# ShuvalovIvan/RayTracingProject

Hardware: AMD Instinct MI355X
Metric: Mrays/sec + frame time, random-spheres 1920x1080x256spp (higher is better)
Workload: dtype f32

## Files before the change

raytracingproject_amd/build.py:

```python
from __future__ import annotations

import os
import subprocess
from concurrent.futures import ThreadPoolExecutor
from pathlib import Path

PKG = Path(__file__).resolve().parent
ROOT = PKG.parent
CSRC = PKG / "csrc"
OBJ = PKG / "build"
LIB = PKG / "lib" / "librt_hip.so"
ARCH = os.environ.get("RT_OFFLOAD_ARCH", "gfx950")
HIPCC = os.environ.get("HIPCC", "/opt/rocm/bin/hipcc")

COMMON = ["-x", "hip", f"--offload-arch={ARCH}", "-O3", "-std=c++17", "-fPIC", "-Wall",
          "-Wno-unused-function", f"-I{ROOT / 'include'}"] + os.environ.get("RT_HIPCC_EXTRA", "").split()
F32_FAST = ["-fno-hip-fp32-correctly-rounded-divide-sqrt", "-fgpu-flush-denormals-to-zero",
            os.environ.get("RT_F32_CONTRACT", "-ffp-contract=on")]
UNITS = {
    "rt_render_f32.hip": F32_FAST,
    "rt_query_grid_f32.hip": F32_FAST,
    "rt_render_f64.hip": ["-ffp-contract=off"],
    "rt_abi.cpp": ["-ffp-contract=off"],
    "rt_plan.cpp": ["-ffp-contract=off"],
# ... 7 lines not shown
HEADERS = ["rt_device.h", "rt_render_impl.h", "rt_occluded.h", "rt_radiance.h", "rt_pixels.h", "rt_moments.h", "rt_aov.h", "rt_scene.h", "rt_launch.h", "rt_bvh.h", "rt_lbvh.h", "rt_ctx.h", "rt_devbuf.h",
           "rt_treelet.h", "rt_pack.h", "rt_batch_cull.h", "rt_denoise.h", "rt_quant.h"]


def _stale(target: Path, deps: list[Path]) -> bool:
    if not target.exists():
        return True
    t = target.stat().st_mtime
    return any(d.stat().st_mtime > t for d in deps)


def _present(p: Path) -> bool:
    try:
        return p.exists()
    except OSError:
        return False


def _compile(src: str, extra: list[str], verbose: bool) -> Path:
    obj = OBJ / (src.rsplit(".", 1)[0] + ".o")
    deps = [CSRC / src] + [CSRC / h for h in HEADERS] + [ROOT / "include" / "rt_hip.h", Path(__file__)]
    if _stale(obj, deps):
        cmd = [HIPCC, *COMMON, *extra, "-c", str(CSRC / src), "-o", str(obj)]
        if verbose:
            print(" ".join(cmd), flush=True)
        subprocess.run(cmd, check=True)
    return obj


def build_native(verbose: bool = False) -> Path:
    OBJ.mkdir(parents=True, exist_ok=True)
    LIB.parent.mkdir(parents=True, exist_ok=True)
    with ThreadPoolExecutor(max_workers=4) as ex:
        objs = list(ex.map(lambda kv: _compile(kv[0], kv[1], verbose), UNITS.items()))
    if _stale(LIB, objs):
        cmd = [HIPCC, f"--offload-arch={ARCH}", "-shared", "-fPIC", "-o", str(LIB), *map(str, objs),
               "-L/opt/rocm/lib", "-lrccl", "-Wl,-rpath,/opt/rocm/lib"]
        if verbose:
            print(" ".join(cmd), flush=True)
        subprocess.run(cmd, check=True)
    return LIB


def build_dropin(verbose: bool = False) -> list[Path]:
    out_dir = ROOT / "examples" / "_build"
    out_dir.mkdir(parents=True, exist_ok=True)
    inc = ROOT / "include" / "rt"
    link = [f"-L{LIB.parent}", "-lrt_hip", f"-Wl,-rpath,{LIB.parent}", "-Wl,-rpath,$ORIGIN/../../raytracingproject_amd/lib"]
    built = []
    for name in ("pixelmatch", "host_queries", "mesh_scene"):
        exe = out_dir / name
        src = ROOT / "examples" / f"{name}.cpp"
        if _stale(exe, [src, LIB, *inc.glob("*.h")]):
            subprocess.run(["g++", "-O2", "-std=c++17", f"-I{inc}", str(src), "-o", str(exe), *link], check=True)
        built.append(exe)
    ref_main = Path("/root/reference/src/main.cpp")
    if _present(ref_main):
        exe = out_dir / "reference_main_on_mi355x"
        if _stale(exe, [ref_main, LIB, *inc.glob("*.h")]):
            with open(ref_main, "rb") as f:
                subprocess.run(["g++", "-O2", "-std=c++17", "-x", "c++", "-", f"-I{inc}", "-o", str(exe), *link],
                               check=True, stdin=f, cwd=inc)
        built.append(exe)
    return built


SAN_FLAGS = ["-O1", "-g", "-fno-omit-frame-pointer", "-fsanitize=address,undefined",
             "-fno-sanitize-recover=all"]
SAN_EXE = OBJ / "san" / "san_driver"
INC = f"-I{ROOT / 'include'}"


def _build_san(exe: Path, srcs: list[Path], deps: list[Path], extra=(), verbose: bool = False) -> Path:
    exe.parent.mkdir(parents=True, exist_ok=True)
    if _stale(exe, [*srcs, *deps, Path(__file__)]):
        cmd = ["g++", "-std=c++17", *SAN_FLAGS, *extra, *map(str, srcs), "-o", str(exe), "-lm"]
        if verbose:
            print(" ".join(cmd), flush=True)
        subprocess.run(cmd, check=True)
    return exe


def build_sanitize(verbose: bool = False) -> Path:
    SAN_EXE.parent.mkdir(parents=True, exist_ok=True)
    orc, oo = ROOT / "oracle" / "rt_oracle.c", SAN_EXE.parent / "rt_oracle.o"
    if _stale(oo, [orc, ROOT / "oracle" / "rt_oracle.h", Path(__file__)]):
        cmd = ["gcc", "-std=c11", *SAN_FLAGS, "-c", str(orc), "-o", str(oo)]
        if verbose:
            print(" ".join(cmd), flush=True)
        subprocess.run(cmd, check=True)
    srcs = [ROOT / "tests" / "cpp" / "sanitize_driver.cpp", CSRC / "rt_obj.cpp", CSRC / "rt_bvh.cpp", oo]
    deps = [CSRC / "rt_bvh.h", CSRC / "rt_scene.h", ROOT / "include" / "rt_hip.h", ROOT / "oracle" / "rt_oracle.h"]
    return _build_san(SAN_EXE, srcs, deps, [INC], verbose)


RESUME_EXE = OBJ / "san" / "grid_resume_driver"
BOXES_EXE = OBJ / "san" / "bvh_boxes_driver"
PACK_EXE = OBJ / "san" / "pack_driver"
DEVBUF_EXE = OBJ / "san" / "devbuf_driver"
BVH_DEPS = [CSRC / "rt_bvh.h", CSRC / "rt_scene.h", ROOT / "include" / "rt_hip.h"]


def build_grid_resume(verbose: bool = False) -> Path:
    srcs = [ROOT / "tests" / "cpp" / "grid_resume_driver.cpp", CSRC / "rt_bvh.cpp"]
    return _build_san(RESUME_EXE, srcs, BVH_DEPS, ["-ffp-contract=off", INC], verbose)


def build_bvh_boxes(verbose: bool = False) -> Path:
    srcs = [ROOT / "tests" / "cpp" / "bvh_boxes_driver.cpp", CSRC / "rt_bvh.cpp"]
    return _build_san(BOXES_EXE, srcs, BVH_DEPS, ["-ffp-contract=off", INC], verbose)


def build_pack(verbose: bool = False) -> Path:
    srcs = [ROOT / "tests" / "cpp" / "pack_driver.cpp", CSRC / "rt_pack.cpp", CSRC / "rt_bvh.cpp"]
    return _build_san(PACK_EXE, srcs, [CSRC / "rt_pack.h", *BVH_DEPS], ["-ffp-contract=off", INC], verbose)


def build_devbuf(verbose: bool = False) -> Path:
    extra = ["-D__HIP_PLATFORM_AMD__", f"-I{CSRC}", "-I/opt/rocm/include"]
    return _build_san(DEVBUF_EXE, [ROOT / "tests" / "cpp" / "devbuf_driver.cpp"], [CSRC / "rt_devbuf.h"], extra, verbose)


QUANT_EXE = OBJ / "san" / "quant_range_driver"


def build_quant_range(verbose: bool = False) -> Path:
    src = ROOT / "tests" / "cpp" / "quant_range_driver.cpp"
    QUANT_EXE.parent.mkdir(parents=True, exist_ok=True)
    if _stale(QUANT_EXE, [src, CSRC / "rt_quant.h", CSRC / "rt_scene.h", Path(__file__)]):
        cmd = ["g++", "-std=c++17", "-O2", "-Wall", "-pthread", f"-I{CSRC}", INC, str(src), "-o", str(QUANT_EXE)]
        if verbose:
            print(" ".join(cmd), flush=True)
        subprocess.run(cmd, check=True)
    return QUANT_EXE


CULL_EXE = OBJ / "san" / "batch_cull_driver"
CULL_MUTANTS = (1, 2, 3)


def build_batch_cull(verbose: bool = False) -> list[Path]:
    src = ROOT / "tests" / "cpp" / "batch_cull_driver.cpp"
    deps = [CSRC / "rt_batch_cull.h", CSRC / "rt_scene.h"]
    exes = [CULL_EXE] + [CULL_EXE.with_name(f"batch_cull_driver_m{m}") for m in CULL_MUTANTS]

    def one(k: int) -> None:
        _build_san(exes[k], [src], deps, ["-O2", "-ffp-contract=off", f"-DRT_CULL_MUTATE={k}", f"-I{CSRC}"], verbose)

    with ThreadPoolExecutor(max_workers=4) as ex:
        list(ex.map(one, range(len(exes))))
    return exes


def build_oracle(verbose: bool = False) -> None:
    oracle = ROOT / "oracle"
    out = None if verbose else subprocess.DEVNULL
    subprocess.run(["make", "-C", str(oracle), "liboracle.so", "rt_oracle_cli", "ref-if-present"], check=True,
                   stdout=out)


if __name__ == "__main__":
    import sys
    if "--sanitize" in sys.argv[1:]:
        print(build_sanitize(verbose=True))
        sys.exit(0)
    print(build_native(verbose=True))
    print(build_dropin(verbose=True))
    build_oracle(verbose=True)
```

raytracingproject_amd/csrc/rt_batch_cull.h:

```cpp
#pragma once
#include <cmath>
#include <cstddef>
#include <cstdint>

#include "rt_scene.h"

namespace rtx {

constexpr int BATCH_CAND_CAP = 24;
constexpr size_t BATCH_CAND_BYTES = 128;
static_assert((BATCH_CAND_CAP + 1) * 4 <= BATCH_CAND_BYTES, "candidate list");

#ifndef RT_CULL_MUTATE
#define RT_CULL_MUTATE 0
#endif
#if RT_CULL_MUTATE == 1
constexpr float CULL_EPS = 0x1p-29f, CULL_EPS_CAM = 0x1p-31f, CULL_UP = 1.f;
#else
constexpr float CULL_EPS = 0x1p-17f, CULL_EPS_CAM = 0x1p-19f, CULL_UP = 1.f + 0x1p-19f;
#endif

struct CullBeam {
    float c[3], ax[3];
    float rl, g, scale;
    bool ok;
};

RT_HD inline CullBeam cull_beam(const float* cam, int defocus, int tx0, int ty0) {
    auto nrm = [](const float* v) { return sqrtf(v[0] * v[0] + v[1] * v[1] + v[2] * v[2]); };
    auto l1 = [](const float* v) { return fabsf(v[0]) + fabsf(v[1]) + fabsf(v[2]); };
    const float* c = cam;
    const float *p00 = cam + 3, *du = cam + 6, *dv = cam + 9, *ddu = cam + 12, *ddv = cam + 15;
    const float fx = (float)tx0 + 3.5f, fy = (float)ty0 + 3.5f;
    CullBeam b;
    float a[3];
    for (int k = 0; k < 3; ++k) {
        b.c[k] = c[k];
        a[k] = (p00[k] + fx * du[k] + fy * dv[k]) - c[k];
    }
    const float L = nrm(a);
    const float iL = 1.f / L;
    for (int k = 0; k < 3; ++k) b.ax[k] = a[k] * iL;
    b.scale = l1(c) + l1(p00) + (fx + 4.5f) * l1(du) + (fy + 4.5f) * l1(dv) + l1(ddu) + l1(ddv);
    const float E = CULL_EPS_CAM * b.scale;
    const float rho = 4.f * (nrm(du) + nrm(dv)) * CULL_UP + E;
#if RT_CULL_MUTATE == 2
    b.rl = E;
#else
    b.rl = (defocus ? nrm(ddu) + nrm(ddv) : 0.f) * CULL_UP + E;
#endif
    const float k = (b.rl + rho) * iL * CULL_UP;
    b.ok = k <= 0.875f;
    b.g = k / (1.f - k) * CULL_UP * CULL_UP;
    return b;
}

RT_HD inline bool cull_keep(const CullBeam& b, const SphereF& s) {
    const float hx = 0.5f * s.cv[0], hy = 0.5f * s.cv[1], hz = 0.5f * s.cv[2];
#if RT_CULL_MUTATE == 3
    const float rb = fabsf(s.r);
#else
    const float rb = fabsf(s.r) + sqrtf(hx * hx + hy * hy + hz * hz) * CULL_UP;
#endif
    const float qx = (s.c[0] + hx) - b.c[0], qy = (s.c[1] + hy) - b.c[1], qz = (s.c[2] + hz) - b.c[2];
    const float qn = sqrtf(qx * qx + qy * qy + qz * qz);
    const float sa = qx * b.ax[0] + qy * b.ax[1] + qz * b.ax[2];
    const float px = qx - sa * b.ax[0], py = qy - sa * b.ax[1], pz = qz - sa * b.ax[2];
    const float perp = sqrtf(px * px + py * py + pz * pz);
    const float W = (rb + b.rl) + CULL_EPS * (qn + b.scale + rb);
    const float bound = (W + b.g * fmaxf(sa + W, 0.f)) * CULL_UP;
    const bool behind = sa < -W, outside = perp > bound;
    return !b.ok || !(behind || outside);
}

RT_HD inline bool batch_cull_keep(const float* cam, int defocus, int tx0, int ty0, const SphereF& s) {
    return cull_keep(cull_beam(cam, defocus, tx0, ty0), s);
}

}
```

raytracingproject_amd/csrc/rt_device.h:

```cpp
#pragma once
#include <type_traits>
#include <hip/hip_runtime.h>

#include <cstdint>

#include "rt_scene.h"
#include "rt_batch_cull.h"
#include "rt_quant.h"


namespace rtx {

__host__ __device__ __forceinline__ uint32_t hash32(uint32_t x) {
    x ^= x >> 16;
    x *= 0x21f0aaadu;
    x ^= x >> 15;
    x *= 0xd35a2d97u;
    x ^= x >> 15;
    return x;
}
__host__ __device__ __forceinline__ uint32_t seed32_of(uint64_t seed) {
    return hash32((uint32_t)seed ^ hash32((uint32_t)(seed >> 32)));
}
constexpr uint32_t RNG_GOLDEN = 0x9e3779b9u;
// ... 35 lines not shown

__device__ __forceinline__ float rcp(float x) { return __builtin_amdgcn_rcpf(x); }
__device__ __forceinline__ double rcp(double x) { return 1.0 / x; }
__device__ __forceinline__ float slab_rcp(float x) { return rcp(x + copysignf(0x1p-100f, x)); }
__device__ __forceinline__ double slab_rcp(double x) { return rcp(x); }

template <class R>
struct V3 {
    R x, y, z;
};
template <class R> __device__ __forceinline__ V3<R> mk(R x, R y, R z) { return V3<R>{x, y, z}; }
template <class R> __device__ __forceinline__ V3<R> operator+(V3<R> a, V3<R> b) { return {a.x + b.x, a.y + b.y, a.z + b.z}; }
template <class R> __device__ __forceinline__ V3<R> operator-(V3<R> a, V3<R> b) { return {a.x - b.x, a.y - b.y, a.z - b.z}; }
template <class R> __device__ __forceinline__ V3<R> operator*(V3<R> a, V3<R> b) { return {a.x * b.x, a.y * b.y, a.z * b.z}; }
template <class R> __device__ __forceinline__ V3<R> operator-(V3<R> a) { return {-a.x, -a.y, -a.z}; }
template <class R> __device__ __forceinline__ V3<R> scl(R t, V3<R> v) { return {t * v.x, t * v.y, t * v.z}; }
template <class R> __device__ __forceinline__ V3<R> dvs(V3<R> v, R t) { return scl(rcp(t), v); }
__device__ __forceinline__ V3<float> madd(float t, V3<float> v, V3<float> c) {
    return {__builtin_fmaf(t, v.x, c.x), __builtin_fmaf(t, v.y, c.y), __builtin_fmaf(t, v.z, c.z)};
}
__device__ __forceinline__ V3<double> madd(double t, V3<double> v, V3<double> c) { return c + scl(t, v); }
template <class R> __device__ __forceinline__ R dot(V3<R> a, V3<R> b) { return a.x * b.x + a.y * b.y + a.z * b.z; }
template <class R> __device__ __forceinline__ V3<R> cross(V3<R> u, V3<R> v) {
    return {u.y * v.z - u.z * v.y, u.z * v.x - u.x * v.z, u.x * v.y - u.y * v.x};
}
template <class R> __device__ __forceinline__ R len2(V3<R> v) { return v.x * v.x + v.y * v.y + v.z * v.z; }
template <class R> __device__ __forceinline__ V3<R> unit(V3<R> v) { return dvs(v, (R)sqrt(len2(v))); }
template <class R> __device__ __forceinline__ V3<R> reflect(V3<R> v, V3<R> n) {
    if constexpr (sizeof(R) == 4) return madd(-2.f * dot(v, n), n, v);
    return v - scl((R)2 * dot(v, n), n);
}
template <class R>
__device__ __forceinline__ V3<R> refract(V3<R> uv, V3<R> n, R e) {
    R cos_theta = fmin(dot(-uv, n), (R)1.0);
    V3<R> perp = scl(e, madd(cos_theta, n, uv));
    V3<R> par = scl(-(R)sqrt(fabs((R)1.0 - len2(perp))), n);
    return perp + par;
}
template <class R, class S> __device__ __forceinline__ V3<R> cvt(V3<S> v) { return {(R)v.x, (R)v.y, (R)v.z}; }
template <class R> __device__ __forceinline__ V3<R> ld3(const double* p) { return {(R)p[0], (R)p[1], (R)p[2]}; }
template <class R> __device__ __forceinline__ V3<R> ld3(const float* p) { return {(R)p[0], (R)p[1], (R)p[2]}; }

constexpr int MAX_PHASES = 8;
struct RenderParams {
    int W, H, spp, max_depth;
    int sample_begin;
    int accumulate;
    int shard, nshards, tiles_x, shard_tiles;
    uint32_t seed32;
    int n_nodes, n_spheres, n_mats, n_big;
    int n_front;
    int stack_size;
    int defocus;
    double cam_center[3], p00[3], du[3], dv[3], ddu[3], ddv[3];
    float f_center[3], f_p00[3], f_du[3], f_dv[3], f_ddu[3], f_ddv[3];
    const Node* nodes;
    const void* spheres;
    const void* mats;
    const SphereD* big;
    const BigF* bigf;
    const Node4* mnodes;
    const void* tris;
    const uint32_t* tmeta;
    int n_mnodes;
    int mstack;
    void* out_sums;
    uint32_t* out_segs;
    unsigned long long* diag;
    void* samples;
    long long* accum;
    uint32_t* accum_flags;
    unsigned long long* accp;
    uint32_t* queue;
    int max_wgs;
    int nph;
    int ph_s0[MAX_PHASES], ph_c[MAX_PHASES], ph_k[MAX_PHASES];
    int coh_refill;
    float box_extent;
    float mbox[6];
    GridHdr grid;
    double tiles_x_inv, tiles_x_inv_half;
    int gsus_lanes, gsus_iters;
    int batch_cap, batch_adopt;
};
constexpr int GSUS_DEFAULT_LANES = 16, GSUS_DEFAULT_ITERS = 8;
constexpr size_t QUEUE_CTRL_BYTES = 4096;
constexpr int FIX_SHIFT = 28;
constexpr int FIX_SAMPLE_SHIFT = 19;
constexpr int FIX_ITEM_SAMPLES = 32;
constexpr int FIX_LAUNCH_SAMPLES = 8191;
constexpr uint32_t FIX_NAN = 1u, FIX_POS = 2u, FIX_NEG = 4u;
__device__ __forceinline__ long long fix_sample(float l, int c, uint32_t& fl, float* r_out = nullptr) {
    constexpr float SC = (float)(1 << FIX_SAMPLE_SHIFT), ISC = 1.f / SC;
    const float r = __builtin_rintf(l * SC);
    if (r_out) *r_out = r;
    const float v = r * ISC;
    if (v == 0.f) return 0;
    const double q = (double)v * (double)(1ll << FIX_SHIFT);
    if (fabs(q) < 0x1p62) return (long long)q;
    fl |= (q != q ? FIX_NAN : q > 0 ? FIX_POS : FIX_NEG) << (3 * c);
    return 0;
}
constexpr int DIAG_SLOTS = 42;

constexpr int COH_FIFO = 128;
template <bool MESH>
struct CohEntryT {
    float t;
    uint32_t pix;
    uint32_t sid;
};
template <>
struct CohEntryT<true> {
    float t;
    uint32_t pix;
    uint32_t sid;
    int32_t id;
};
using CohEntry = CohEntryT<false>;
static_assert(sizeof(CohEntryT<false>) == 12 && sizeof(CohEntryT<true>) == 16, "CohEntry");
template <bool MESH>
struct CohEntryD {
    double t;
    uint32_t pix;
    uint32_t sid;
};
template <>
struct CohEntryD<true> {
    double t;
    uint32_t pix;
    uint32_t sid;
    int32_t id;
    uint32_t pad;
};
static_assert(sizeof(CohEntryD<false>) == 16 && sizeof(CohEntryD<true>) == 24, "CohEntryD");
#ifndef RT_FIFO_RNG0
#define RT_FIFO_RNG0 1
#endif
#ifndef RT_CAM_ONEBASE
#define RT_CAM_ONEBASE 1
#endif
#ifndef RT_LEAN_FINISH
#define RT_LEAN_FINISH 1
#endif
#ifndef RT_SCATTER_PROLOGUE
#define RT_SCATTER_PROLOGUE 1
#endif
#ifndef RT_BATCH_ONEADOPT
#define RT_BATCH_ONEADOPT 1
#endif
#ifndef RT_POP_THROUGH
#define RT_POP_THROUGH 1
#endif
struct alignas(16) CohEntryR {
    float t;
    uint32_t pix;
    uint32_t sid;
    uint32_t rng0;
};
static_assert(sizeof(CohEntryR) == 16 && alignof(CohEntryR) == 16, "CohEntryR");
template <class R, bool MESH, bool RNG0> struct CohEntrySel { using type = CohEntryT<MESH>; };
template <bool MESH, bool RNG0> struct CohEntrySel<double, MESH, RNG0> { using type = CohEntryD<MESH>; };
template <> struct CohEntrySel<float, false, true> { using type = CohEntryR; };
template <class R, bool MESH, bool RNG0 = false> using CohEntryX = typename CohEntrySel<R, MESH, RNG0>::type;
constexpr size_t COH_SUM_BYTES = 64 * 3 * sizeof(float);
constexpr size_t COH_PARK_BYTES = 64 * 4 * sizeof(float);
constexpr size_t coh_wave_bytes(bool mesh, bool sums, int fifo = COH_FIFO, bool f64 = false, bool park = false,
                                bool cand = false) {
    const size_t entry = f64                    ? (mesh ? sizeof(CohEntryD<true>) : sizeof(CohEntryD<false>))
                         : cand && RT_FIFO_RNG0 ? sizeof(CohEntryR)
                                                : (mesh ? sizeof(CohEntryT<true>) : sizeof(CohEntryT<false>));
    return (size_t)fifo * entry +
           (sums && !f64 ? COH_SUM_BYTES : 0) + (park ? COH_PARK_BYTES : 0) + (cand ? BATCH_CAND_BYTES : 0);
}
constexpr size_t COH_WAVE_BYTES = coh_wave_bytes(false, true);
struct CohConst {
    float cam[18];
    int nph;
    int ph_s0[MAX_PHASES], ph_c[MAX_PHASES], ph_k[MAX_PHASES];
    int pad;
};
static_assert(sizeof(CohConst) % 16 == 0, "CohConst");
constexpr size_t COH_CAM_BYTES = sizeof(CohConst);


template <class R> struct Prec;
template <> struct Prec<float> { using Sph = SphereF; using Mat = MatF; using Tri = TriF; };
template <> struct Prec<double> { using Sph = SphereD; using Mat = MatD; using Tri = TriD; };

template <class R>
struct SceneView {
    const Node* nodes;
    const typename Prec<R>::Sph* sph;
    const typename Prec<R>::Mat* mat;
    const SphereD* big;
    const BigF* bigf;
    int n_nodes, n_big, n_front;
    const Node4* mnodes;
    const typename Prec<R>::Tri* tris;
    const uint32_t* tmeta;
    int n_mnodes;
    uint32_t* mstack;
    int n_mstack;
    float mbox[6];
    GridHdr grid;
    const __attribute__((address_space(4))) GridHdr* gridp;
    float box_extent;
};

template <class R>
struct Ray {
    V3<R> o, d;
    R time;
};

template <class T, bool EXACT, bool SELECT = false>
__device__ __forceinline__ bool sphere_root(V3<T> c, T r, V3<T> cv, bool moving, V3<T> o, V3<T> d, T a, T inv_a,
                                            T time, T tmin, T tmax, bool self, T& t) {
    V3<T> center = c;
    if (EXACT) {
        if (moving) center = c + scl(time, cv);
    } else {
        center = madd(time, cv, c);
    }
    if (EXACT) {
        V3<T> oc = o - center;
        T half_b = dot(oc, d);
        T cc = len2(oc) - r * r;
        T disc = half_b * half_b - a * cc;
        if (disc < 0) return false;
        T sq = (T)sqrt(disc);
        T root = (-half_b - sq) / a;
        if (!(tmin < root && root < tmax)) {
            root = (-half_b + sq) / a;
            if (!(tmin < root && root < tmax)) return false;
        }
        t = root;
        return true;
    }
    const V3<T> f = o - center;
    const T b = -dot(f, d);
    T root;
    if (self) {
        root = (T)2 * b * inv_a;
        if (!(tmin < root && root < tmax)) return false;
        t = root;
        return true;
    }
    const V3<T> l = madd(b * inv_a, d, f);
    const T r2 = r * r;
    const T disc = r2 - len2(l);
    if (disc < 0) return false;
    const T cc = len2(f) - r2;
    const T q = b + copysign((T)sqrt(a * disc), b);
    const T ta = cc * rcp(q), tb = q * inv_a;
    const T t0 = fmin(ta, tb), t1 = fmax(ta, tb);
    if (SELECT) {
        root = (tmin < t0 && t0 < tmax) ? t0 : t1;
        t = root;
        return tmin < root && root < tmax;
    }
    root = t0;
    if (!(tmin < root && root < tmax)) {
        root = t1;
        if (!(tmin < root && root < tmax)) return false;
    }
    t = root;
    return true;
}

template <class T>
__device__ __forceinline__ bool tri_root(V3<T> v0, V3<T> e1, V3<T> e2, V3<T> o, V3<T> d, T tmin, T tmax, T& t) {
    constexpr T EPS = (T)0;
    const V3<T> pv = cross(d, e2);
    const T det = dot(e1, pv);
    if (det == (T)0) return false;
    const T inv_det = rcp(det);
    const V3<T> tv = o - v0;
    const T u = dot(tv, pv) * inv_det;
    if (u < -EPS || u > (T)1 + EPS) return false;
    const V3<T> qv = cross(tv, e1);
    const T v = dot(d, qv) * inv_det;
    if (v < -EPS || u + v > (T)1 + EPS) return false;
    const T tt = dot(e2, qv) * inv_det;
    if (!(tmin < tt && tt < tmax)) return false;
    t = tt;
    return true;
}

__device__ __forceinline__ void vfence(float& x) { asm volatile("" : "+v"(x)); }
__device__ __forceinline__ bool tri_wt(V3<float> p0, V3<float> p1, V3<float> p2, V3<float> n, V3<float> o,
                                       V3<float> d, float tmin, float tmax, float& t) {
    const float nd = dot(n, d);
    float Ax, Ay, Az;
    {
#pragma clang fp contract(off)
        Ax = p0.x - o.x, Ay = p0.y - o.y, Az = p0.z - o.z;
    }
    const float tt = dot(n, mk(Ax, Ay, Az)) * rcp(nd);
    if (!(tmin < tt && tt < tmax)) return false;
    auto outside = [nd](float e) { return nd > 0.f ? e < 0.f : e > 0.f; };
    {
#pragma clang fp contract(off)
        const float Bx = p1.x - o.x, By = p1.y - o.y, Bz = p1.z - o.z;
        float ec = d.x * (Ay * Bz - Az * By) + d.y * (Az * Bx - Ax * Bz) + d.z * (Ax * By - Ay * Bx);
        vfence(ec);
// ... 56 lines not shown
    double tn = fmax(fmax(fmin(t0x, t1x), fmin(t0y, t1y)), fmax(fmin(t0z, t1z), tmin));
    double tf = fmin(fmin(fmax(t0x, t1x), fmax(t0y, t1y)), fmin(fmax(t0z, t1z), tmax));
    tnear = tn;
    return tn <= tf;
}

struct ConsSlabs {
    float f[3], clo[3], chi[3];
};
__device__ __forceinline__ ConsSlabs cons_slabs(V3<double> o, V3<double> d, float extent) {
    ConsSlabs s;
    const double oo[3] = {o.x, o.y, o.z}, dd[3] = {d.x, d.y, d.z};
#pragma unroll
    for (int a = 0; a < 3; ++a) {
        if (fabs(dd[a]) < 0x1p-60) {
            s.f[a] = 0.f;
            s.clo[a] = -__builtin_huge_valf();
            s.chi[a] = __builtin_huge_valf();
            continue;
        }
        const float f = (float)(1.0 / dd[a]);
        const float m = (float)((fabs(oo[a]) + (double)extent) * 0x1p-21 * fabs((double)f));
        const float c = -((float)oo[a] * f);
        s.f[a] = f;
        s.clo[a] = f > 0.f ? c - m : c + m;
        s.chi[a] = f > 0.f ? c + m : c - m;
    }
    return s;
}
__device__ __forceinline__ bool box_hit_cons(const float lo[3], const float hi[3], const ConsSlabs& s, float tmin,
                                             float tmax, float& tnear) {
    const float t0x = __builtin_fmaf(lo[0], s.f[0], s.clo[0]), t1x = __builtin_fmaf(hi[0], s.f[0], s.chi[0]);
    const float t0y = __builtin_fmaf(lo[1], s.f[1], s.clo[1]), t1y = __builtin_fmaf(hi[1], s.f[1], s.chi[1]);
    const float t0z = __builtin_fmaf(lo[2], s.f[2], s.clo[2]), t1z = __builtin_fmaf(hi[2], s.f[2], s.chi[2]);
    const float tn = fmaxf(fmaxf(fminf(t0x, t1x), fminf(t0y, t1y)), fmaxf(fminf(t0z, t1z), tmin));
    const float tf = fminf(fminf(fmaxf(t0x, t1x), fmaxf(t0y, t1y)), fmaxf(t0z, t1z));
    tnear = tn;
    return tn <= tf && tn <= tmax;
}
constexpr float CONS_TMIN = 0.0009f;
__device__ __forceinline__ float cons_tmax(double tmax) { return (float)tmax * (1.f + 0x1p-22f); }

enum { TRAV_SELROOT = 8, TRAV_B128 = 16, TRAV_F32BOX = 32, TRAV_COH = 64, TRAV_NOSUM = 128, TRAV_TBIN = 256,
       TRAV_CULL = 512, TRAV_PERSIST = 2048, TRAV_MTOP = 4096, TRAV_MIFIF = 8192, TRAV_MWHILE = 16384,
       TRAV_MQ = 32768, TRAV_GRID = 65536, TRAV_GFLAT = 131072,
       TRAV_G3D = 262144 };
constexpr int TRAV_REMOVED = TRAV_TBIN | TRAV_MTOP;
constexpr int coh_fifo_entries(int) { return COH_FIFO; }
constexpr bool coh_parks(bool mesh, int tr, bool f64) { return mesh && !f64 && (tr & TRAV_GRID) != 0; }
constexpr bool coh_cands(bool mesh, int tr, bool f64) { return !mesh && !f64 && (tr & TRAV_GRID) != 0; }
constexpr bool coh_adopts(bool mesh, int tr, bool f64) { return coh_cands(mesh, tr, f64); }
constexpr bool coh_rng0(bool mesh, int tr, bool f64) { return RT_FIFO_RNG0 && coh_cands(mesh, tr, f64); }
constexpr bool coh_cam1(bool mesh, int tr, bool f64) { return RT_CAM_ONEBASE && coh_cands(mesh, tr, f64); }
constexpr bool coh_lean(bool mesh, int tr, bool f64) { return RT_LEAN_FINISH && coh_cands(mesh, tr, f64); }
constexpr bool coh_refl1(bool mesh, int tr, bool f64) {
    return RT_SCATTER_PROLOGUE && coh_cands(mesh, tr, f64) && (tr & TRAV_GFLAT) != 0;
}
constexpr bool coh_adopt1(bool mesh, int tr, bool f64) { return RT_BATCH_ONEADOPT && coh_cands(mesh, tr, f64); }
constexpr bool coh_popthru(bool mesh, int tr, bool f64) { return RT_POP_THROUGH && coh_cands(mesh, tr, f64); }
typedef __attribute__((address_space(3))) const uint32_t lds_cu32;
typedef __attribute__((address_space(3))) const float4 lds_cf4;
__device__ __forceinline__ void keep_live(uint32_t v) { asm volatile("" ::"v"(v)); }
template <class R, bool EXACT, bool DIAG = false, int TRAV = 0, bool MESH = false, bool SUSP = false,
          bool CAND = false>
__device__ __forceinline__ Hit<R> closest_hit(const SceneView<R>& sc, const Ray<R>& ray, uint16_t* stack, int stride,
                                              int self_id, DiagCounters* dg = nullptr, float* resume = nullptr,
                                              const Hit<R>* part = nullptr, int sus_lanes = 0, int sus_iters = 0,
                                              uint32_t clist = 0, int ncand = 0) {
    static_assert(!SUSP || (!EXACT && !MESH && (TRAV & TRAV_GRID) != 0 && (TRAV & TRAV_GFLAT) != 0),
                  "resumable walks: the fp32 sphere-only flat grid walk");
    static_assert(!CAND || (!SUSP && coh_cands(MESH, TRAV, EXACT)), "candidate lists: the fp32 sphere-grid kernels");
    constexpr R TMIN = (R)0.001;
    Hit<R> h;
    h.id = -1;
    h.td = __builtin_huge_val();
    R tmax = (R)__builtin_huge_valf();
    const V3<R> o = ray.o, d = ray.d;
    const R a = len2(d);
    const R inv_a = rcp(a);
    [[maybe_unused]] bool resumed = false;
    [[maybe_unused]] float t_from = -1.f;
    if constexpr (SUSP) {
        t_from = *resume;
        *resume = -1.f;
        resumed = t_from >= 0.f;
        if (resumed) {
            h.id = part->id;
            tmax = part->t;
        }
    }

    if (SUSP && resumed) {
    } else if (EXACT) {
        const V3<double> od = cvt<double>(o), dd = cvt<double>(d);
        double tmaxd = __builtin_huge_val();
        for (int k = 0; k < sc.n_big; ++k) {
            const SphereD& s = sc.big[k];
            double t;
            if (sphere_root<double, true>(mk(s.c[0], s.c[1], s.c[2]), s.r, mk(s.cv[0], s.cv[1], s.cv[2]),
                                          (s.meta >> 30) & 1u, od, dd, (double)a, 0.0, (double)ray.time, 0.001,
                                          tmaxd, false, t)) {
                tmaxd = t;
                h.id = -2 - k;
                h.td = t;
            }
        }
        if (h.id != -1) tmax = (R)h.td;
    } else {
        for (int k = 0; k < sc.n_big; ++k) {
            const BigF& s = sc.bigf[k];
            V3<R> p0 = mk((R)s.p0[0], (R)s.p0[1], (R)s.p0[2]);
            if ((s.meta >> 30) & 1u) p0 = madd((R)ray.time, mk((R)s.cv[0], (R)s.cv[1], (R)s.cv[2]), p0);
            const V3<R> q = o - p0, nn = mk((R)s.n[0], (R)s.n[1], (R)s.n[2]);
            const R b = -fma((R)s.r, dot(nn, d), dot(q, d));
            R t;
            if ((-2 - k) == self_id) {
                t = (R)2 * b * inv_a;
                if (!(TMIN < t && t < tmax)) continue;
            } else {
                const R cc = fma((R)2 * (R)s.r, dot(nn, q), dot(q, q));
                const R disc = b * b - a * cc;
                if (disc < 0) continue;
                const R qq = b + copysign((R)sqrt(disc), b);
                const R ta = cc * rcp(qq), tb = qq * inv_a;
                const R t0 = fmin(ta, tb), t1 = fmax(ta, tb);
                t = t0;
                if (!(TMIN < t && t < tmax)) {
                    t = t1;
                    if (!(TMIN < t && t < tmax)) continue;
                }
            }
            tmax = t;
            h.id = -2 - k;
        }
    }

    using Sph = typename Prec<R>::Sph;
    auto test_rec = [&](const Sph* rec, bool is_self, R tlim, R& tk) -> bool {
        if constexpr (!EXACT && (TRAV & TRAV_B128) != 0) {
            const float4* q = (const float4*)rec;
            const float4 s0 = q[0], s1 = q[1];
            keep_live(__float_as_uint(s0.w));
            keep_live(__float_as_uint(s1.w));
            return sphere_root<R, false, (TRAV & TRAV_SELROOT) != 0>(
                mk((R)s0.x, (R)s0.y, (R)s0.z), (R)s0.w, mk((R)s1.x, (R)s1.y, (R)s1.z), false, o, d, a, inv_a,
                ray.time, TMIN, tlim, is_self, tk);
        }
        const auto& s = *rec;
        return sphere_root<R, EXACT, (TRAV & TRAV_SELROOT) != 0>(mk((R)s.c[0], (R)s.c[1], (R)s.c[2]), (R)s.r,
                                     mk((R)s.cv[0], (R)s.cv[1], (R)s.cv[2]), (s.meta >> 30) & 1u, o, d, a, inv_a,
                                     ray.time, TMIN, tlim, !EXACT && is_self, tk);
    };
    auto test_one = [&](int k, R tlim, R& tk) -> bool { return test_rec(sc.sph + k, k == self_id, tlim, tk); };
    if constexpr (CAND) {
        uint32_t hit_off = 0xffffffffu;
        for (int i = 0; i < ncand; ++i) {
            if (DIAG) DiagCounters::count(dg->leaf_it, dg->leaf_act), ++dg->steps;
            const uint32_t off = (uint32_t)__builtin_amdgcn_readfirstlane(
                (int)*(const lds_cu32*)(uintptr_t)(clist + 4u * (uint32_t)i));
            const Sph* rec = (const Sph*)(const float4*)(const lds_cf4*)(uintptr_t)off;
            R t;
            if (test_rec(rec, false, tmax, t)) {
                tmax = t;
                hit_off = off;
            }
        }
        if (hit_off != 0xffffffffu)
            h.id = (int)((hit_off - (uint32_t)sc.n_nodes * (uint32_t)sizeof(Node)) / (uint32_t)sizeof(Sph));
        h.t = tmax;
        return h;
    }
    for (int k = 0; k < (SUSP && resumed ? 0 : sc.n_front); ++k) {
        R t;
        if (test_one(k, tmax, t)) {
            tmax = t;
            h.id = k;
        }
    }

    if constexpr ((TRAV & TRAV_GRID) != 0) {
        if (sc.n_nodes > 0) {
            constexpr bool FLAT = (TRAV & TRAV_GFLAT) != 0;
            const GridHdr g = [&]() {
                if constexpr (!MESH) {
                    auto gp = sc.gridp;
                    asm volatile("" : "+s"(gp));
                    return *(const GridHdr*)gp;
                } else {
                    return sc.grid;
                }
            }();
            const uint32_t pad = (uint32_t)g.res[0] * (uint32_t)g.res[1];
            const uint32_t* cells = (const uint32_t*)sc.nodes + pad;
            const unsigned char* lbase = (const unsigned char*)sc.nodes;
            const uint32_t sph0 = (uint32_t)sc.n_nodes * (uint32_t)sizeof(Node);
            const uint32_t self_off = self_id >= 0 && self_id < MESH_HIT_BASE
                                          ? sph0 + (uint32_t)self_id * (uint32_t)sizeof(Sph)
                                          : 0xffffffffu;
            uint32_t hit_off = 0xffffffffu;
            const float INF = __builtin_huge_valf();
            const V3<float> of = cvt<float>(o), df = cvt<float>(d);
            float tn, tf, nx, ny = INF, nz, dtx, dty = 0.f, dtz;
            int ci;
            {
                const V3<float> inv = mk(slab_rcp(df.x), slab_rcp(df.y), slab_rcp(df.z));
                const V3<float> oi = of * inv;
                const float tm = (float)ray.time;
                const int sk = tm >= 0.f && tm <= 1.f ? min((int)(tm * g.slab_k), g.n_slab - 1) : g.n_slab;
                const float2* sbx = (const float2*)(lbase + g.slab_off) + sk;
                const int sst = g.n_slab + 1;
                const float2 bx = sbx[0], by = sbx[sst], bz = sbx[2 * sst];
                const float t0x = fmaf(bx.x, inv.x, -oi.x), t1x = fmaf(bx.y, inv.x, -oi.x);
                const float t0y = fmaf(by.x, inv.y, -oi.y), t1y = fmaf(by.y, inv.y, -oi.y);
                const float t0z = fmaf(bz.x, inv.z, -oi.z), t1z = fmaf(bz.y, inv.z, -oi.z);
                tn = fmaxf(fmaxf(fminf(t0x, t1x), fminf(t0y, t1y)), fmaxf(fminf(t0z, t1z), (float)TMIN));
                tf = fminf(fminf(fmaxf(t0x, t1x), fmaxf(t0y, t1y)), fminf(fmaxf(t0z, t1z), (float)tmax));
                if constexpr (SUSP) tn = fmaxf(tn, t_from);
                auto axis = [&](int a, float oa, float da, float iv, float oia, float& n, float& dt) {
                    int i = (int)((fmaf(tn, da, oa) - g.lo[a]) * g.inv_cs[a]);
                    i = i < 0 ? 0 : (i >= g.res[a] ? g.res[a] - 1 : i);
                    const float plane = fmaf((float)(da > 0.f ? i + 1 : i), g.cs[a], g.lo[a]);
                    n = da != 0.f ? fmaf(plane, iv, -oia) : INF;
                    dt = g.cs[a] * fabsf(iv);
                    return i;
                };
                const int ix = axis(0, of.x, df.x, inv.x, oi.x, nx, dtx);
                const int iz = axis(2, of.z, df.z, inv.z, oi.z, nz, dtz);
                if constexpr (FLAT) {
                    ci = iz * g.res[0] + ix;
                } else {
                    const int iy = axis(1, of.y, df.y, inv.y, oi.y, ny, dty);
                    ci = (iz * g.res[1] + iy) * g.res[0] + ix;
                }
            }
            if (tn <= tf) {
                const int sy = g.res[0], sz = g.res[1] * sy;
                const int stx = df.x > 0.f ? 1 : -1, sty = df.y > 0.f ? sy : -sy, stz = df.z > 0.f ? sz : -sz;
                [[maybe_unused]] uint32_t ca = (uint32_t)(uintptr_t)(cells + ci);
                [[maybe_unused]] const int sx4 = stx * 4, sz4 = stz * 4;
                uint32_t w = FLAT ? *(const lds_cu32*)(uintptr_t)ca : cells[ci];
                uint32_t cur = w & GRID_POS_MASK, end = w >> GRID_POS_BITS;
                if constexpr (!SUSP) {
                    for (;;) {
                        if (cur >= end) {
                            if (DIAG) DiagCounters::count(dg->inner_it, dg->inner_act), ++dg->steps;
                            if constexpr (FLAT) {
                                const bool bx = nx <= nz;
                                const float te = bx ? nx : nz;
                                if (!(te < (float)tmax && te < tf)) break;
                                ca += bx ? sx4 : sz4;
                                nx = bx ? nx + dtx : nx;
                                nz = bx ? nz : nz + dtz;
                            } else {
                                const float te = fminf(fminf(nx, ny), nz);
                                if (!(te < (float)tmax && te < tf)) break;
                                const bool bx = nx == te, by = !bx && ny == te, bz = !bx && !by;
                                ci += bx ? stx : (by ? sty : stz);
                                nx = bx ? nx + dtx : nx;
                                ny = by ? ny + dty : ny;
                                nz = bz ? nz + dtz : nz;
                            }
                            w = FLAT ? *(const lds_cu32*)(uintptr_t)ca : cells[ci];
                            cur = w & GRID_POS_MASK;
                            end = w >> GRID_POS_BITS;
                        }
                        if (cur < end) {
                            if (DIAG) DiagCounters::count(dg->leaf_it, dg->leaf_act), ++dg->steps;
                            const uint32_t off = *(const lds_cu32*)(uintptr_t)cur;
                            cur += 4u;
                            R t;
                            const Sph* rec = (const Sph*)(const float4*)(const lds_cf4*)(uintptr_t)off;
                            if (test_rec(rec, off == self_off, tmax, t)) {
                                tmax = t;
                                hit_off = off;
                            }
                        }
                    }
                } else {
                    const int entered = __builtin_amdgcn_readfirstlane((int)__popcll(__ballot(1)));
                    int block = sus_iters;
                    for (;;) {
                        int left = __builtin_amdgcn_readfirstlane(block);
                        for (;;) {
                            if (cur >= end) {
                                if (DIAG) DiagCounters::count(dg->inner_it, dg->inner_act), ++dg->steps;
                                const bool bx = nx <= nz;
                                const float te = bx ? nx : nz;
                                if (!(te < (float)tmax && te < tf)) break;
                                ca += bx ? sx4 : sz4;
                                nx = bx ? nx + dtx : nx;
                                nz = bx ? nz : nz + dtz;
                                w = *(const lds_cu32*)(uintptr_t)ca;
                                cur = w & GRID_POS_MASK;
                                end = w >> GRID_POS_BITS;
                            }
                            if (cur < end) {
                                if (DIAG) DiagCounters::count(dg->leaf_it, dg->leaf_act), ++dg->steps;
                                const uint32_t off = *(const lds_cu32*)(uintptr_t)cur;
                                cur += 4u;
                                R t;
                                const Sph* rec = (const Sph*)(const float4*)(const lds_cf4*)(uintptr_t)off;
                                if (test_rec(rec, off == self_off, tmax, t)) {
                                    tmax = t;
                                    hit_off = off;
                                }
                            }
                            if constexpr (DIAG)
// ... 518 lines not shown
```

raytracingproject_amd/csrc/rt_render_impl.h:

```cpp
#pragma once
#include "rt_device.h"
#include "rt_launch.h"

namespace rtx {

__device__ __forceinline__ V3<float> mul_rn(V3<float> a, V3<float> b) {
#pragma clang fp contract(off)
    return {a.x * b.x, a.y * b.y, a.z * b.z};
}
__device__ __forceinline__ V3<float> add_rn(V3<float> a, V3<float> b) {
#pragma clang fp contract(off)
    return {a.x + b.x, a.y + b.y, a.z + b.z};
}
__device__ __forceinline__ V3<double> mul_rn(V3<double> a, V3<double> b) { return a * b; }
__device__ __forceinline__ V3<double> add_rn(V3<double> a, V3<double> b) { return a + b; }

__device__ __forceinline__ void copy16(void* dst, const void* src, size_t bytes, int tid, int nthreads) {
    uint4* d = (uint4*)dst;
    const uint4* s = (const uint4*)src;
    const size_t n = bytes / 16;
    for (size_t k = (size_t)tid; k < n; k += (size_t)nthreads) d[k] = s[k];
}

constexpr uint32_t ITEM_NONE = 0xffffffffu;
// ... 344 lines not shown
            return camera_ray<R>(P, px, py, rr);
        else
            return camera_ray_lds<coh_cam1(MESH, TRAV, EXACT)>(cam, P.defocus, px, py, rr, kdef, kout);
    };
    constexpr int FIFO = coh_fifo_entries(TRAV);
    const int lane = threadIdx.x & 63;
    constexpr bool CAND = coh_cands(MESH, TRAV, EXACT);
    constexpr bool RNG0 = coh_rng0(MESH, TRAV, EXACT);
    using Entry = CohEntryX<R, MESH, RNG0>;
    [[maybe_unused]] uint32_t* const clist =
        (uint32_t*)((unsigned char*)fifo + (size_t)FIFO * sizeof(Entry) + (SUMS ? COH_SUM_BYTES : 0));
    DiagCounters dg, dgb;
    unsigned long long n_bounce = 0, n_live = 0, cyc_trav = 0, cyc_shade = 0, cyc_batch = 0, n_paths = 0, n_seg = 0,
                       n_batch = 0, n_pop = 0;
    const unsigned long long t_start = DIAG ? __builtin_amdgcn_s_memtime() : 0;
    const unsigned long long rt_start = DIAG ? __builtin_amdgcn_s_memrealtime() : 0;
    unsigned long long rt_dry = 0, n_drain = 0;
    unsigned long long n_in_item = 0, n_direct = 0, n_item_flush = 0;

    uint32_t head = 0, count = 0;
    ItemDec cur = decode_item(P, P, ITEM_NONE);
    int bi = 0;
    bool dry = false;
    if (SUMS) isum[lane] = isum[64 + lane] = isum[128 + lane] = 0.f;

    bool elig = false;
    constexpr bool LEAN = coh_lean(MESH, TRAV, EXACT);
    [[maybe_unused]] bool direct_here = false;
    [[maybe_unused]] unsigned long long n_shade_pass = 0, n_pass_direct = 0, n_pass_mixed = 0;
    auto finish = [&](uint32_t pp, bool in_item, V3<R> L, uint32_t sg, uint32_t srel) {
        if constexpr (EXACT) {
            R* o = samp + ((size_t)srel * npx_all + pp) * 3;
            o[0] = L.x;
            o[1] = L.y;
            o[2] = L.z;
            if (P.out_segs && sg) atomicAdd(P.out_segs + pp, sg);
            return;
        }
        const float qx = __builtin_rintf(L.x * SC) * ISC, qy = __builtin_rintf(L.y * SC) * ISC,
                    qz = __builtin_rintf(L.z * SC) * ISC;
        if constexpr (LEAN) {
            if (rtx::in01(qx, qy, qz)) {
                if (SUMS && in_item) {
                    const uint32_t q = pp & 63u;
                    if (qx != 0.f) atomicAdd(isum + q, qx);
                    if (qy != 0.f) atomicAdd(isum + 64 + q, qy);
                    if (qz != 0.f) atomicAdd(isum + 128 + q, qz);
                    if (DIAG) ++n_in_item;
                } else {
                    const uint32_t ux = (uint32_t)(qx * SC), uy = (uint32_t)(qy * SC), uz = (uint32_t)(qz * SC);
                    const unsigned long long prg = (unsigned long long)ux | (unsigned long long)uy << 32;
                    if (prg) atomicAdd(P.accp + (size_t)pp * 2, prg);
                    if (uz) atomicAdd(P.accp + (size_t)pp * 2 + 1, (unsigned long long)uz);
                    if (DIAG) ++n_direct, direct_here = true;
                }
                if (P.out_segs && sg) atomicAdd(P.out_segs + pp, sg);
            } else {
                flush_sample(P, pp, qx, qy, qz, sg);
                if (DIAG) ++n_direct, direct_here = true;
            }
            if (DIAG) ++n_paths;
            return;
        }
        const bool in01 = qx >= 0.f && qx <= 1.f && qy >= 0.f && qy <= 1.f && qz >= 0.f && qz <= 1.f;
        if (SUMS && in_item && in01) {
            const uint32_t q = pp & 63u;
            if (qx != 0.f) atomicAdd(isum + q, qx);
            if (qy != 0.f) atomicAdd(isum + 64 + q, qy);
            if (qz != 0.f) atomicAdd(isum + 128 + q, qz);
            if (P.out_segs && sg) atomicAdd(P.out_segs + pp, sg);
            if (DIAG) ++n_in_item;
        } else {
            flush_sample(P, pp, qx, qy, qz, sg);
            if (DIAG) ++n_direct, direct_here = true;
        }
        if (DIAG) ++n_paths;
    };

    bool live = false, ready = false, fin = false;
    constexpr bool SUSP = !EXACT && !MESH && (TR & TRAV_GRID) != 0 && (TR & TRAV_GFLAT) != 0;
    [[maybe_unused]] float tres = -1.f;
    [[maybe_unused]] unsigned long long n_susp = 0;
    uint32_t pix = 0;
    uint32_t psid = 0;
    V3<R> thr = mk((R)1, (R)1, (R)1);
    [[maybe_unused]] V3<R> att_stack[EXACT ? 64 : 1];
    CounterRng rng;
    rng.st = 0;
    int nsc = 0, self = NO_SELF;
    constexpr bool PARK = coh_parks(MESH, TRAV, EXACT);
    [[maybe_unused]] float* const park =
        (float*)((unsigned char*)fifo + (size_t)FIFO * sizeof(Entry) + (SUMS ? COH_SUM_BYTES : 0)) + lane;
    auto park_thr = [&]() -> V3<R> { return mk((R)park[0], (R)park[64], (R)park[128]); };
    auto park_nsc = [&]() -> int { return __float_as_int(park[192]); };
    auto park_set = [&](V3<R> t, int n) {
        park[0] = (float)t.x;
        park[64] = (float)t.y;
        park[128] = (float)t.z;
        park[192] = __int_as_float(n);
    };
    Ray<R> ray;
    ray.o = ray.d = thr;
    ray.time = (R)0;
    Hit<R> h;
    h.t = (R)0;
    h.td = 0.0;
    h.id = -1;

    constexpr bool ADOPT = coh_adopts(MESH, TRAV, EXACT);
    static_assert(!ADOPT || (!PARK && !EXACT), "adopted hits: the fp32 sphere-only grid kernels");
    constexpr bool ADOPT1 = ADOPT && coh_adopt1(MESH, TRAV, EXACT);
    constexpr bool POP_THRU = ADOPT1 && coh_popthru(MESH, TRAV, EXACT);
    [[maybe_unused]] unsigned long long n_adopt = 0, n_pop_pass = 0, n_pop_lanes = 0;
    [[maybe_unused]] unsigned long long n_pass_hist[8] = {};
    [[maybe_unused]] bool after_adopt = false;
    auto batch = [&]([[maybe_unused]] const bool need) {
        const unsigned long long tb = DIAG ? __builtin_amdgcn_s_memtime() : 0;
        if constexpr (DIAG && ADOPT) after_adopt = false;
        if (bi >= cur.c) {
            if (SUMS && cur.lt >= 0) {
                const float fx = isum[lane], fy = isum[64 + lane], fz = isum[128 + lane];
                if (fx != 0.f || fy != 0.f || fz != 0.f) {
                    flush_sample(P, (uint32_t)cur.lt * 64u + (uint32_t)lane, fx, fy, fz, 0u, (float)cur.c);
                    if (DIAG) ++n_item_flush;
                }
                isum[lane] = isum[64 + lane] = isum[128 + lane] = 0.f;
            }
            cur = decode_item(P, kc, fetch_item(P, kc));
            bi = 0;
            elig = false;
            if (cur.lt < 0) {
                dry = true;
                if (DIAG) rt_dry = __builtin_amdgcn_s_memrealtime();
                return;
            }
            if constexpr (CAND) {
                const int cap = P.batch_cap;
                uint32_t n = 0xffffffffu;
                if (cap > 0) {
                    const CullBeam bm = cull_beam(cam, P.defocus, cur.tx0, cur.ty0);
                    const int nsph = P.n_spheres;
                    const uint32_t sph0 = (uint32_t)sc.n_nodes * (uint32_t)sizeof(Node);
                    n = 0;
                    for (int b0 = 0; b0 < nsph; b0 += 64) {
                        const int k = b0 + lane;
                        const bool keep = k < nsph && cull_keep(bm, sc.sph[k]);
                        const unsigned long long km = __ballot(keep);
                        const uint32_t r = n + __builtin_amdgcn_mbcnt_hi((uint32_t)(km >> 32),
                                                                         __builtin_amdgcn_mbcnt_lo((uint32_t)km, 0u));
                        if (keep && r < (uint32_t)BATCH_CAND_CAP) clist[r] = sph0 + (uint32_t)k * (uint32_t)sizeof(SphereF);
                        n += (uint32_t)__popcll(km);
                    }
                    if (n > (uint32_t)cap) n = 0xffffffffu;
                }
                if (lane == 0) clist[BATCH_CAND_CAP] = n;
                __builtin_amdgcn_wave_barrier();
            }
        }
        const int s = cur.s0 + bi++;
        int bl = lane;
        if constexpr (ADOPT1) asm volatile("" : "+v"(bl));
        const int px = cur.tx0 + (bl & 7), py = cur.ty0 + (bl >> 3);
        const uint32_t pp = (uint32_t)cur.lt * 64u + (uint32_t)lane;
        bool hit = false;
        [[maybe_unused]] bool adopt = false;
        Hit<R> hb;
        hb.t = (R)0;
        hb.id = -1;
        [[maybe_unused]] int kd = 15;
        [[maybe_unused]] uint32_t rng0 = 0;
        if constexpr (ADOPT1) {
            const bool valid = px < P.W && py < P.H && P.max_depth > 0;
            Ray<R> pr;
            [[maybe_unused]] CounterRng r2;
            if (valid) {
                r2.start(hash32(P.seed32 ^ (uint32_t)(py * P.W + px)), (uint32_t)s);
                if constexpr (RNG0) rng0 = r2.st;
                pr = KDEF ? cam_ray(px, py, r2, -1, &kd) : cam_ray(px, py, r2);
                const int nc = __builtin_amdgcn_readfirstlane((int)clist[BATCH_CAND_CAP]);
                if (nc >= 0)
                    hb = closest_hit<R, EXACT, DIAG, TR, MESH, false, true>(sc, pr, stack, BLOCK, NO_SELF, &dgb, nullptr,
                                                                            nullptr, 0, 0, (uint32_t)(uintptr_t)clist, nc);
                else
                    hb = closest_hit<R, EXACT, DIAG, TR, MESH>(sc, pr, stack, BLOCK, NO_SELF, &dgb);
            }
            hit = hb.id != -1;
            if (valid && !hit) finish(pp, true, sky(pr.d), 1u, (uint32_t)(s - P.sample_begin));
            adopt = hit && need && P.batch_adopt;
            if (adopt) {
                ray = pr;
                if constexpr (RNG0) {
                    rng.st = rng0;
                    rng.skip(3u + (P.defocus ? 2u * (uint32_t)kd + 2u : 0u));
                } else {
                    rng = r2;
                }
                h.t = hb.t;
                h.td = (double)hb.t;
                h.id = hb.id;
                pix = pp;
                thr = mk((R)1, (R)1, (R)1);
                nsc = 0;
                self = NO_SELF;
                live = ready = true;
                elig = true;
                if (DIAG) ++n_adopt;
            }
        } else if (px < P.W && py < P.H && P.max_depth > 0) {
            CounterRng r2;
            r2.start(hash32(P.seed32 ^ (uint32_t)(py * P.W + px)), (uint32_t)s);
            if constexpr (RNG0) rng0 = r2.st;
            const Ray<R> pr = KDEF ? cam_ray(px, py, r2, -1, &kd) : cam_ray(px, py, r2);
            if constexpr (CAND) {
                const int nc = __builtin_amdgcn_readfirstlane((int)clist[BATCH_CAND_CAP]);
                if (nc >= 0)
                    hb = closest_hit<R, EXACT, DIAG, TR, MESH, false, true>(sc, pr, stack, BLOCK, NO_SELF, &dgb, nullptr,
                                                                            nullptr, 0, 0, (uint32_t)(uintptr_t)clist, nc);
                else
                    hb = closest_hit<R, EXACT, DIAG, TR, MESH>(sc, pr, stack, BLOCK, NO_SELF, &dgb);
            } else {
                hb = closest_hit<R, EXACT, DIAG, TR, MESH>(sc, pr, stack, BLOCK, NO_SELF, &dgb);
            }
            if (hb.id == -1) {
                finish(pp, true, sky(pr.d), 1u, (uint32_t)(s - P.sample_begin));
            } else {
                hit = true;
                if constexpr (ADOPT) {
                    if (need && P.batch_adopt) {
                        adopt = true;
                        ray = pr;
                        if constexpr (RNG0) {
                            rng.st = rng0;
                            rng.skip(3u + (P.defocus ? 2u * (uint32_t)kd + 2u : 0u));
                        } else {
                            rng = r2;
                        }
                        h.t = hb.t;
                        h.td = (double)hb.t;
                        h.id = hb.id;
                        pix = pp;
                        thr = mk((R)1, (R)1, (R)1);
                        nsc = 0;
                        self = NO_SELF;
                        live = ready = true;
                        elig = true;
                        if (DIAG) ++n_adopt;
                    }
                }
            }
        } else if constexpr (EXACT) {
            finish(pp, true, mk((R)0, (R)0, (R)0), 0u, (uint32_t)(s - P.sample_begin));
        }
        const bool push = ADOPT ? hit && !adopt : hit;
        const unsigned long long hm = __ballot(push);
        if (push) {
            const uint32_t r = __builtin_amdgcn_mbcnt_hi((uint32_t)(hm >> 32), __builtin_amdgcn_mbcnt_lo((uint32_t)hm, 0u));
            Entry e;
            e.t = hb.t;
            e.pix = pp;
            if constexpr (RNG0) e.rng0 = rng0;
            if constexpr (MESH) {
                e.sid = (uint32_t)(s - P.sample_begin);
                if constexpr (KDEF) e.sid |= (uint32_t)min(kd, 15) << 28;
                e.id = hb.id;
            } else {
                e.sid = (uint32_t)(s - P.sample_begin) | ((uint32_t)(hb.id + 16) << 16);
                if constexpr (KDEF) e.sid |= (uint32_t)min(kd, 15) << 28;
            }
            fifo[(head + count + r) & (FIFO - 1)] = e;
        }
        count += (uint32_t)__popcll(hm);
        if constexpr (DIAG && ADOPT) after_adopt = __ballot(adopt) != 0;
        if (DIAG && lane == 0) {
            ++n_batch;
            cyc_batch += __builtin_amdgcn_s_memtime() - tb;
        }
    };

    auto sky_L = [&]() -> V3<R> {
        if constexpr (EXACT) {
            V3<R> L = sky(ray.d);
            for (int k = nsc - 1; k >= 0; --k) L = att_stack[k] * L;
            return L;
        } else if constexpr (PARK) {
            return mul_rn(park_thr(), sky(ray.d));
        } else {
            return mul_rn(thr, sky(ray.d));
        }
    };

    for (;;) {
        if constexpr (LAUNDER) Pp = kernarg();
        const unsigned long long tsh = DIAG ? __builtin_amdgcn_s_memtime() : 0;
        for (;;) {
            if (ready && h.id == -1) {
                ready = false;
                if constexpr (PARK)
                    finish(pix, elig, sky_L(), (uint32_t)park_nsc() + 1u, psid);
                else
                    finish(pix, elig, sky_L(), (uint32_t)nsc + 1u, psid);
                live = false;
            }
            for (;;) {
                bool need = !fin && !live;
                unsigned long long m = __ballot(need);
                if (m == 0) break;
// ... 510 lines not shown
```

Baseline: 21470.

## Sort batch candidate spheres by conservative near distance and early-exit traversal

After the per-tile beam culling builds the candidate sphere list, each candidate gets a conservative lower bound on hit distance. That bound is packed with the sphere index into one word, and the list is rank-sorted within the wave. The candidate loop then visits spheres in near-to-far order and stops once every lane's current tmax is below the next candidate's bound, which skips far sphere tests. Ties by index are kept by nudging tlim, which preserves the original hit choice. The cost is extra per-tile work for the bounds and an O(n) readlane ranking, plus a dependence on the bound being truly conservative.

```diff
diff --git a/raytracingproject_amd/build.py b/raytracingproject_amd/build.py
--- a/raytracingproject_amd/build.py
+++ b/raytracingproject_amd/build.py
@@ -183,6 +183,23 @@
     return exes
 
 
+DEPTH_EXE = OBJ / "san" / "cand_depth_driver"
+DEPTH_MUTANTS = (1, 2, 3, 4)
+
+
+def build_cand_depth(verbose: bool = False) -> list[Path]:
+    src = ROOT / "tests" / "cpp" / "cand_depth_driver.cpp"
+    deps = [CSRC / "rt_batch_cull.h", CSRC / "rt_scene.h"]
+    exes = [DEPTH_EXE] + [DEPTH_EXE.with_name(f"cand_depth_driver_m{m}") for m in DEPTH_MUTANTS]
+
+    def one(k: int) -> None:
+        _build_san(exes[k], [src], deps, ["-O2", "-ffp-contract=off", f"-DRT_CULL_MUTATE={k}", f"-I{CSRC}"], verbose)
+
+    with ThreadPoolExecutor(max_workers=4) as ex:
+        list(ex.map(one, range(len(exes))))
+    return exes
+
+
 def build_oracle(verbose: bool = False) -> None:
     oracle = ROOT / "oracle"
     out = None if verbose else subprocess.DEVNULL
diff --git a/raytracingproject_amd/csrc/rt_batch_cull.h b/raytracingproject_amd/csrc/rt_batch_cull.h
--- a/raytracingproject_amd/csrc/rt_batch_cull.h
+++ b/raytracingproject_amd/csrc/rt_batch_cull.h
@@ -2,6 +2,7 @@
 #include <cmath>
 #include <cstddef>
 #include <cstdint>
+#include <cstring>
 
 #include "rt_scene.h"
 
@@ -16,14 +17,18 @@
 #endif
 #if RT_CULL_MUTATE == 1
 constexpr float CULL_EPS = 0x1p-29f, CULL_EPS_CAM = 0x1p-31f, CULL_UP = 1.f;
+constexpr float CULL_SQ = 0x1p-20f, CULL_DN = 1.f;
 #else
 constexpr float CULL_EPS = 0x1p-17f, CULL_EPS_CAM = 0x1p-19f, CULL_UP = 1.f + 0x1p-19f;
+constexpr float CULL_SQ = 0x1p-8f, CULL_DN = 1.f - 0x1p-19f;
 #endif
+constexpr uint32_t CAND_IDX_BITS = 12, CAND_IDX_MASK = (1u << CAND_IDX_BITS) - 1u;
 
 struct CullBeam {
     float c[3], ax[3];
     float rl, g, scale;
     bool ok;
+    float nd;
 };
 
 RT_HD inline CullBeam cull_beam(const float* cam, int defocus, int tx0, int ty0) {
@@ -52,6 +57,7 @@
     const float k = (b.rl + rho) * iL * CULL_UP;
     b.ok = k <= 0.875f;
     b.g = k / (1.f - k) * CULL_UP * CULL_UP;
+    b.nd = iL / ((1.f + k) * CULL_UP * CULL_UP);
     return b;
 }
 
@@ -73,6 +79,43 @@
     return !b.ok || !(behind || outside);
 }
 
+RT_HD inline float cull_near(const CullBeam& b, const SphereF& s) {
+    const float hx = 0.5f * s.cv[0], hy = 0.5f * s.cv[1], hz = 0.5f * s.cv[2];
+#if RT_CULL_MUTATE == 3
+    const float rb = fabsf(s.r);
+#else
+    const float rb = fabsf(s.r) + sqrtf(hx * hx + hy * hy + hz * hz) * CULL_UP;
+#endif
+    const float qx = (s.c[0] + hx) - b.c[0], qy = (s.c[1] + hy) - b.c[1], qz = (s.c[2] + hz) - b.c[2];
+    const float qn = sqrtf(qx * qx + qy * qy + qz * qz);
+    const float sa = qx * b.ax[0] + qy * b.ax[1] + qz * b.ax[2];
+    const float W = (rb + b.rl) + CULL_EPS * (qn + b.scale + rb);
+    const float G = CULL_SQ * sqrtf(rb * (qn + b.scale + rb));
+    const float near = ((sa - W) - G) * b.nd * CULL_DN;
+    return b.ok && near > 0.f ? near : 0.f;
+}
+
+RT_HD inline uint32_t cand_pack(float near, uint32_t k) {
+    uint32_t u;
+    memcpy(&u, &near, 4);
+#if RT_CULL_MUTATE == 4
+    u += CAND_IDX_MASK;
+#endif
+    return (u & ~CAND_IDX_MASK) | k;
+}
+RT_HD inline float cand_near(uint32_t w) {
+    w &= ~CAND_IDX_MASK;
+    float f;
+    memcpy(&f, &w, 4);
+    return f;
+}
+RT_HD inline uint32_t cand_index(uint32_t w) { return w & CAND_IDX_MASK; }
+RT_HD inline uint32_t cand_rank(const uint32_t* words, uint32_t n, uint32_t w) {
+    uint32_t r = 0;
+    for (uint32_t j = 0; j < n; ++j) r += words[j] < w;
+    return r;
+}
+
 RT_HD inline bool batch_cull_keep(const float* cam, int defocus, int tx0, int ty0, const SphereF& s) {
     return cull_keep(cull_beam(cam, defocus, tx0, ty0), s);
 }
diff --git a/raytracingproject_amd/csrc/rt_device.h b/raytracingproject_amd/csrc/rt_device.h
--- a/raytracingproject_amd/csrc/rt_device.h
+++ b/raytracingproject_amd/csrc/rt_device.h
@@ -211,6 +211,9 @@
 #ifndef RT_POP_THROUGH
 #define RT_POP_THROUGH 1
 #endif
+#ifndef RT_CAND_DEPTH
+#define RT_CAND_DEPTH 1
+#endif
 struct alignas(16) CohEntryR {
     float t;
     uint32_t pix;
@@ -573,7 +576,28 @@
                                      ray.time, TMIN, tlim, !EXACT && is_self, tk);
     };
     auto test_one = [&](int k, R tlim, R& tk) -> bool { return test_rec(sc.sph + k, k == self_id, tlim, tk); };
-    if constexpr (CAND) {
+    if constexpr (CAND && RT_CAND_DEPTH) {
+        static_assert((TRAV & TRAV_B128) != 0 && (TRAV & TRAV_SELROOT) != 0, "the coh_cands kernels' sphere test");
+        const uint32_t sph0 = (uint32_t)sc.n_nodes * (uint32_t)sizeof(Node);
+        uint32_t hit_k = 0;
+        for (int i = 0; i < ncand; ++i) {
+            const uint32_t w = (uint32_t)__builtin_amdgcn_readfirstlane(
+                (int)*(const lds_cu32*)(uintptr_t)(clist + 4u * (uint32_t)i));
+            if (!__builtin_amdgcn_ballot_w64(tmax >= __uint_as_float(w & ~CAND_IDX_MASK))) break;
+            if (DIAG) DiagCounters::count(dg->leaf_it, dg->leaf_act), ++dg->steps;
+            const uint32_t k1 = (w & CAND_IDX_MASK) + 1u;
+            const Sph* rec = (const Sph*)(const float4*)(const lds_cf4*)(uintptr_t)(sph0 + (k1 - 1u) * (uint32_t)sizeof(Sph));
+            const R tlim = __uint_as_float(__float_as_uint(tmax) + (k1 < hit_k ? 1u : 0u));
+            R t;
+            if (test_rec(rec, false, tlim, t)) {
+                tmax = t;
+                hit_k = k1;
+            }
+        }
+        if (hit_k) h.id = (int)hit_k - 1;
+        h.t = tmax;
+        return h;
+    } else if constexpr (CAND) {
         uint32_t hit_off = 0xffffffffu;
         for (int i = 0; i < ncand; ++i) {
             if (DIAG) DiagCounters::count(dg->leaf_it, dg->leaf_act), ++dg->steps;
diff --git a/raytracingproject_amd/csrc/rt_render_impl.h b/raytracingproject_amd/csrc/rt_render_impl.h
--- a/raytracingproject_amd/csrc/rt_render_impl.h
+++ b/raytracingproject_amd/csrc/rt_render_impl.h
@@ -520,6 +520,22 @@
                         n += (uint32_t)__popcll(km);
                     }
                     if (n > (uint32_t)cap) n = 0xffffffffu;
+                    if constexpr (RT_CAND_DEPTH) {
+                        static_assert(MAX_LEAF_FIRST + MAX_BIG <= (int)CAND_IDX_MASK, "list word: 12 index bits");
+                        if (n <= (uint32_t)BATCH_CAND_CAP) {
+                            __builtin_amdgcn_wave_barrier();
+                            const bool has = (uint32_t)lane < n;
+                            uint32_t w = 0xffffffffu;
+                            if (has) {
+                                const uint32_t k = (clist[lane] - sph0) / (uint32_t)sizeof(SphereF);
+                                w = cand_pack(cull_near(bm, sc.sph[k]), k);
+                            }
+                            uint32_t r = 0;
+                            for (uint32_t j = 0; j < n; ++j) r += (uint32_t)__builtin_amdgcn_readlane((int)w, (int)j) < w;
+                            __builtin_amdgcn_wave_barrier();
+                            if (has) clist[r] = w;
+                        }
+                    }
                 }
                 if (lane == 0) clist[BATCH_CAND_CAP] = n;
                 __builtin_amdgcn_wave_barrier();
```

Result: faster. 21700, median of 6 (+1.1%).
